# panbanda/islands

Measured on AMD Instinct MI355X. Metric: queries/sec @ recall@10>=0.95, 10Mx768 ef=128, higher is better.
Workload: dtype f32; 1 GPU; 10000000 x 768 f32 rows resident in HBM (in-memory provider), hierarchical Gaussian mixture, graph by the harness (tools/synth.py::build_graph: k-means medoid levels flattened into one layer, diversified links, parent->child and reverse edges), deg<= 60 (mean 38.6), query batch 1024, k=10, ef=128, cosine; nodes=10000000, dim=768, query_batch=1024, k=10, ef=128, graph=harness, distinct_leaves=False, parallelism=single, searches_in_flight=32, distinct_batches=497, replayed_queries=1688

## Files before the change

### include/islands_amd.h

```cpp
#ifndef ISLANDS_AMD_H
#define ISLANDS_AMD_H

#include <stddef.h>
#include <stdint.h>

#ifdef __cplusplus
extern "C" {
#endif

#define ISL_ABI_VERSION 3

typedef int32_t isl_status;

enum {
  ISL_OK = 0,
  ISL_ERR_DIMENSION_MISMATCH = 1,
  ISL_ERR_EMPTY_COLLECTION = 2,
  ISL_ERR_INVALID_CONFIG = 3,
  ISL_ERR_INDEX_NOT_BUILT = 4,
  ISL_ERR_NODE_NOT_FOUND = 5,
  ISL_ERR_SERIALIZATION = 6,
  ISL_ERR_DESERIALIZATION = 7,
  ISL_ERR_IO = 8,
  ISL_ERR_HNSW = 9,
// ... 126 lines not shown
  uint64_t expansions;
  uint64_t edges;
  uint64_t evals;
  uint64_t pushes;
  uint64_t exact_path;
  uint64_t replayed;
  double kernel_ms;
  uint64_t encoded_nodes;
  uint64_t recompute_rounds;
  uint64_t allocations;
} isl_search_stats;

isl_status isl_index_prepare(isl_index* idx, uint64_t max_nq, uint64_t max_ef, uint64_t max_k,
                             int32_t lanes);

isl_status isl_search_batch(const isl_index* idx, const float* queries, uint64_t nq, uint64_t d,
                            uint64_t k, uint64_t ef, uint64_t* out_ids, float* out_dist,
                            uint32_t* out_count);
isl_status isl_search_batch_async(const isl_index* idx, const float* queries, uint64_t nq, uint64_t d,
                                  uint64_t k, uint64_t ef, uint64_t* out_ids, float* out_dist,
                                  uint32_t* out_count, uint64_t* token);
isl_status isl_search_batch_device(const isl_index* idx, const float* d_queries, uint64_t nq,
                                   uint64_t d, uint64_t k, uint64_t ef, uint64_t* d_out_ids,
                                   float* d_out_dist, uint32_t* d_out_count, void* stream);
isl_status isl_search_batch_device_async(const isl_index* idx, const float* d_queries, uint64_t nq,
                                         uint64_t d, uint64_t k, uint64_t ef, uint64_t* d_out_ids,
                                         float* d_out_dist, uint32_t* d_out_count, void* stream,
                                         uint64_t* token);
isl_status isl_search_wait_stats(const isl_index* idx, uint64_t token, isl_search_stats* stats);
isl_status isl_search_wait(const isl_index* idx, uint64_t token);
isl_status isl_search_stream_wait(const isl_index* idx, uint64_t token, void* stream);
isl_status isl_index_group_counters(const isl_index* idx, uint64_t* launches, uint64_t* shared_launches,
                                    uint64_t* shared_calls);
isl_status isl_search(const isl_index* idx, const float* query, uint64_t d, uint64_t k,
                      uint64_t* out_ids, float* out_dist, uint32_t* out_count);

isl_status isl_search_last_stats(const isl_index* idx, isl_search_stats* out);

#define ISL_MAX_ENTRY_SEEDS 65536ull
isl_status isl_index_select_entry_seeds(isl_index* idx, uint64_t count, uint64_t* out_ids, uint64_t* out_count);
isl_status isl_index_set_entry_seeds(isl_index* idx, const uint64_t* ids, uint64_t count);
isl_status isl_index_entry_seeds(const isl_index* idx, uint64_t* out, uint64_t cap, uint64_t* count);
isl_status isl_index_pick_entries(const isl_index* idx, const float* queries, uint64_t nq, uint64_t d,
                                  uint64_t* out_ids, int32_t mem, void* stream);

isl_status isl_distance(int32_t metric, const float* a, uint64_t na, const float* b, uint64_t nb,
                        float* out);
isl_status isl_distance_squared(int32_t metric, const float* a, uint64_t na, const float* b,
                                uint64_t nb, float* out);
isl_status isl_distance_batch(int32_t metric, const float* query, uint64_t d, const float* rows,
                              uint64_t n, uint64_t row_len, float* out, int32_t mem, int32_t device,
                              void* stream);
isl_status isl_normalize_rows(float* rows, uint64_t n, uint64_t d, int32_t mem, int32_t device,
                              void* stream);

isl_status isl_distance_matrix(int32_t metric, const float* queries, uint64_t nq, const float* rows,
                               uint64_t n, uint64_t d, float* out, int32_t mem, int32_t device,
                               void* stream);
isl_status isl_bruteforce_topk(int32_t metric, const float* queries, uint64_t nq, const float* rows,
                               uint64_t n, uint64_t d, uint64_t k, uint64_t* out_ids, float* out_dist,
                               uint32_t* out_count, int32_t mem, int32_t device, void* stream);

isl_status isl_merge_topk(uint64_t nlists, uint64_t nq, uint64_t k, const uint64_t* ids,
                          const float* scores, const uint32_t* counts, const uint64_t* id_base,
                          uint64_t top_k, uint64_t* out_ids, float* out_scores,
                          uint32_t* out_src, uint32_t* out_count, int32_t mem, int32_t device,
// ... 159 lines not shown
```

### islands_amd/_ffi.py

```python
from __future__ import annotations

import ctypes as C
import os

os.environ.setdefault("GPU_MAX_HW_QUEUES", "32")

_HERE = os.path.dirname(os.path.abspath(__file__))
LIB_PATH = os.environ.get("ISL_AMD_LIB") or os.path.join(_HERE, "lib", "libislands_amd.so")

u64, u32, i32, f32 = C.c_uint64, C.c_uint32, C.c_int32, C.c_float
P = C.POINTER


class LeannConfigC(C.Structure):
    _fields_ = [
        ("m", u64), ("m0", u64), ("ef_construction", u64), ("ml", C.c_double),
        ("max_layers", u64), ("metric", u32), ("ef_search", u64), ("beam_width", u64),
        ("prune_ratio", f32), ("pruning_strategy", u32), ("high_degree_pruning", C.c_uint8),
        ("hub_percentile", f32), ("is_compact", C.c_uint8), ("is_recompute", C.c_uint8),
    ]


class BertConfigC(C.Structure):
    _fields_ = [("vocab_size", u32), ("hidden", u32), ("layers", u32), ("heads", u32),
# ... 46 lines not shown
    "isl_index_len": (u64, [C.c_void_p]),
    "isl_index_is_empty": (i32, [C.c_void_p]),
    "isl_index_dimension": (i32, [C.c_void_p, P(u64)]),
    "isl_index_storage_bytes": (u64, [C.c_void_p]),
    "isl_index_is_recompute": (i32, [C.c_void_p]),
    "isl_index_is_compact": (i32, [C.c_void_p]),
    "isl_index_config": (i32, [C.c_void_p, P(LeannConfigC)]),
    "isl_index_entry_point": (i32, [C.c_void_p, P(u64)]),
    "isl_index_max_level": (u64, [C.c_void_p]),
    "isl_index_get_neighbors": (i32, [C.c_void_p, u64, P(P(u64)), P(C.c_size_t)]),
    "isl_index_upload": (i32, [C.c_void_p, i32]),
    "isl_set_embeddings": (i32, [C.c_void_p, C.c_void_p, u64, u64, i32, i32]),
    "isl_search_batch": (i32, [C.c_void_p, C.c_void_p, u64, u64, u64, u64, C.c_void_p,
                               C.c_void_p, C.c_void_p]),
    "isl_hnsw_from_bytes": (i32, [C.c_void_p, C.c_size_t, i32, P(C.c_void_p)]),
    "isl_distance_matrix_bf16": (i32, [i32, C.c_void_p, u64, C.c_void_p, u64, u64, C.c_void_p, i32, i32,
                                       C.c_void_p]),
    "isl_index_set_pq_codes": (i32, [C.c_void_p, C.c_void_p, C.c_void_p, u64, i32]),
    "isl_search_two_level_batch": (i32, [C.c_void_p, C.c_void_p, u64, u64, u64, u64, C.c_float,
                                         C.c_void_p, C.c_void_p, C.c_void_p]),
    "isl_search_two_level_batch_device": (i32, [C.c_void_p, C.c_void_p, u64, u64, u64, u64,
                                                C.c_float, C.c_void_p, C.c_void_p, C.c_void_p,
                                                C.c_void_p]),
    "isl_search_two_level_batch_device_async": (i32, [C.c_void_p, C.c_void_p, u64, u64, u64, u64,
                                                      C.c_float, C.c_void_p, C.c_void_p, C.c_void_p,
                                                      C.c_void_p, P(u64)]),
    "isl_search_batch_device": (i32, [C.c_void_p, C.c_void_p, u64, u64, u64, u64, C.c_void_p,
                                      C.c_void_p, C.c_void_p, C.c_void_p]),
    "isl_search_batch_device_async": (i32, [C.c_void_p, C.c_void_p, u64, u64, u64, u64, C.c_void_p,
                                            C.c_void_p, C.c_void_p, C.c_void_p, P(u64)]),
    "isl_search_wait": (i32, [C.c_void_p, u64]),
    "isl_search_stream_wait": (i32, [C.c_void_p, u64, C.c_void_p]),
    "isl_index_group_counters": (i32, [C.c_void_p, P(u64), P(u64), P(u64)]),
    "isl_shard_record_bytes": (u64, [u64, u64]),
    "isl_merge_topk_packed_async": (i32, [u64, u64, u64, C.c_void_p, u64, C.c_void_p, u64, C.c_void_p, C.c_void_p,
                                          C.c_void_p, C.c_void_p, C.c_void_p, i32, C.c_void_p]),
    "isl_shard_unique_id": (i32, [C.c_void_p]),
    "isl_shard_group_create": (i32, [i32, i32, i32, C.c_void_p, P(C.c_void_p)]),
    "isl_shard_group_create_host": (i32, [i32, i32, i32, C.c_void_p, C.c_void_p, P(C.c_void_p)]),
    "isl_shard_group_info": (i32, [C.c_void_p, P(i32), P(i32), P(i32), P(i32)]),
    "isl_shard_group_free": (None, [C.c_void_p]),
    "isl_sharded_searcher_new": (i32, [C.c_void_p, C.c_void_p, u64, C.c_void_p, i32, P(C.c_void_p)]),
    "isl_sharded_searcher_free": (None, [C.c_void_p]),
    "isl_sharded_prepare": (i32, [C.c_void_p, u64, u64, u64]),
    "isl_sharded_submit": (i32, [C.c_void_p, C.c_void_p, u64, u64, u64, u64, C.c_void_p, P(u64)]),
    "isl_sharded_result": (i32, [C.c_void_p, u64, P(C.c_void_p), P(C.c_void_p), P(C.c_void_p), P(C.c_void_p),
                                 P(SearchStatsC)]),
    "isl_sharded_search_batch": (i32, [C.c_void_p, C.c_void_p, u64, u64, u64, u64, C.c_void_p, C.c_void_p,
                                       C.c_void_p, C.c_void_p]),
    "isl_sharded_flags": (i32, [C.c_void_p, P(u32)]),
    "isl_search_wait_stats": (i32, [C.c_void_p, u64, P(SearchStatsC)]),
    "isl_search_batch_async": (i32, [C.c_void_p, C.c_void_p, u64, u64, u64, u64, C.c_void_p,
                                     C.c_void_p, C.c_void_p, P(u64)]),
    "isl_index_prepare": (i32, [C.c_void_p, u64, u64, u64, i32]),
    "isl_search": (i32, [C.c_void_p, C.c_void_p, u64, u64, C.c_void_p, C.c_void_p, C.c_void_p]),
    "isl_search_last_stats": (i32, [C.c_void_p, P(SearchStatsC)]),
    "isl_distance": (i32, [i32, C.c_void_p, u64, C.c_void_p, u64, P(f32)]),
    "isl_distance_squared": (i32, [i32, C.c_void_p, u64, C.c_void_p, u64, P(f32)]),
    "isl_distance_batch": (i32, [i32, C.c_void_p, u64, C.c_void_p, u64, u64, C.c_void_p, i32, i32,
                                 C.c_void_p]),
    "isl_normalize_rows": (i32, [C.c_void_p, u64, u64, i32, i32, C.c_void_p]),
    "isl_distance_matrix": (i32, [i32, C.c_void_p, u64, C.c_void_p, u64, u64, C.c_void_p, i32, i32,
                                  C.c_void_p]),
    "isl_bruteforce_topk": (i32, [i32, C.c_void_p, u64, C.c_void_p, u64, u64, u64, C.c_void_p,
                                  C.c_void_p, C.c_void_p, i32, i32, C.c_void_p]),
    "isl_row_sumsq_bf16": (i32, [C.c_void_p, u64, u64, C.c_void_p, i32, i32, C.c_void_p]),
# ... 99 lines not shown
```

### islands_amd/csrc/common.hpp

```cpp
#pragma once

#include <hip/hip_runtime.h>

#include <algorithm>
#include <cstdarg>
#include <cstdint>
#include <cstdlib>
#include <cstdio>
#include <cstring>
#include <atomic>
#include <chrono>
#include <mutex>
#include <string>
#include <thread>
#include <type_traits>
#include <vector>

#include "../../include/islands_amd.h"
#include "device_buffer.hpp"
#include "row_table.hpp"

namespace isl {

struct ErrorRecord {
// ... 24 lines not shown
  switch (metric) {
    case ISL_METRIC_COSINE: f(std::integral_constant<int, ISL_METRIC_COSINE>{}); break;
    case ISL_METRIC_EUCLIDEAN: f(std::integral_constant<int, ISL_METRIC_EUCLIDEAN>{}); break;
    case ISL_METRIC_DOT: f(std::integral_constant<int, ISL_METRIC_DOT>{}); break;
    default: f(std::integral_constant<int, ISL_METRIC_MANHATTAN>{}); break;
  }
}

isl_status use_device(int32_t device);
int device_cu_count(int32_t device);

struct SearchWorkspace {
  uint32_t slots = 0;
  uint32_t ovf_bits = 0;
  DeviceBuffer<uint32_t> ovf_tab;
  DeviceBuffer<uint32_t> status;
  DeviceBuffer<uint64_t> payload;
  DeviceBuffer<uint32_t> ctr;
  DeviceBuffer<uint32_t> ticket;
  DeviceBuffer<uint32_t> redo;
  DeviceBuffer<uint32_t> replay;
  DeviceBuffer<uint32_t> qsel;
  DeviceBuffer<uint32_t> qsel_h;
  DeviceBuffer<uint64_t> plog;
  DeviceBuffer<float> q_stage;
  DeviceBuffer<uint64_t> ids_stage;
  DeviceBuffer<float> dist_stage;
  DeviceBuffer<uint32_t> count_stage;
  PinnedBuffer<float> h_q;
  PinnedBuffer<uint64_t> h_ids;
  PinnedBuffer<float> h_dist;
  PinnedBuffer<uint32_t> h_count;
  hipStream_t stream = nullptr;
  hipEvent_t ev0 = nullptr, ev1 = nullptr, ev_in = nullptr, ev_done = nullptr;
  bool busy = false;
  bool waiting = false;
  bool enqueued = false;
  bool ticket_clean = false;
  bool publish_results = false;
  uint64_t token = 0;
  uint64_t nq_inflight = 0, k_inflight = 0;
  uint32_t ef_inflight = 0;
  bool fast_inflight = false;
  hipStream_t st_inflight = nullptr;
  uint64_t* u_ids = nullptr;
  float* u_dist = nullptr;
  uint32_t* u_count = nullptr;
  PinnedBuffer<uint32_t> h_status;
  PinnedBuffer<uint32_t> h_ctr;
  PinnedBuffer<uint32_t> h_head;
  DeviceBuffer<uint64_t> d_prof;
  DeviceBuffer<uint64_t> d_tline;
  DeviceBuffer<uint32_t> q_entry;
  DeviceBuffer<float> co_q;
  DeviceBuffer<uint64_t> co_ids;
  DeviceBuffer<float> co_dist;
  DeviceBuffer<uint32_t> co_cnt;
  DeviceBuffer<uint32_t> miss;
  DeviceBuffer<uint32_t> uniq;
  DeviceBuffer<uint32_t> uniq_count;
  uint64_t miss_cap = 0;
  uint64_t pref_cap = 0;
  DeviceBuffer<uint32_t> qstate;
  DeviceBuffer<uint32_t> qflag;
  DeviceBuffer<uint32_t> qlist;
  PinnedBuffer<uint32_t> h_qlist;
  DeviceBuffer<uint32_t> uslots;
  DeviceBuffer<uint32_t> xslot;
  PinnedBuffer<uint32_t> h_xlist;
  DeviceBuffer<float> tl_tables;
  std::thread* worker = nullptr;
  bool threaded = false;
  isl_status worker_status = ISL_OK;
  ErrorRecord worker_error;
  uint64_t alloc_events = 0;
  uint64_t alloc_mark = 0;
  isl_search_stats stats{};
  bool grp = false;
  SearchWorkspace* grp_launch = nullptr;
  uint32_t grp_offset = 0;
  hipEvent_t grp_ready = nullptr;
  uint64_t grp_allocs = 0;
  bool grp_failed = false;
  isl_status grp_status = ISL_OK;
  ErrorRecord grp_error;
  int32_t pool_lane = -1;
  bool union_launch = false;
  PinnedBuffer<uint64_t> h_members;
  DeviceBuffer<uint32_t> grp_scratch;
};

constexpr int kSearchLanes = 32;

int hw_queues_at_load();
constexpr int kGroupBelowQueues = 8;
struct GroupSwitches { bool off; uint32_t cap, room; };
inline GroupSwitches group_switches() {
  auto num = [](const char* name) -> uint32_t {
    const char* e = getenv(name);
    const long long v = e ? atoll(e) : 0;
    return v > 0 ? (uint32_t)std::min<long long>(v, 0x7FFFFFFF) : 0u;
  };
  const char* off = getenv("ISL_NO_GROUP");
  const bool is_off = (off && *off) ? strcmp(off, "0") != 0 : hw_queues_at_load() >= kGroupBelowQueues;
  return GroupSwitches{is_off, num("ISL_GROUP_CAP"), num("ISL_GROUP_ROOM")};
}
struct GroupState;

struct ExactPool {
  uint32_t slots = 0;
  uint64_t cand_cap = 0;
  DeviceBuffer<float> cand_d;
  DeviceBuffer<uint32_t> cand_id;
  DeviceBuffer<uint32_t> vis_bits;
  uint64_t vis_words = 0;
  DeviceBuffer<uint32_t> ulist;
  uint32_t ulist_cap = 0;
  DeviceBuffer<uint32_t> locks;
  DeviceBuffer<uint32_t> xstate;
  uint32_t xstate_words = 0;
// ... 122 lines not shown
```

### islands_amd/csrc/search.hip

```cpp
#include "search_geometry.hpp"
#include "search_internal.hpp"

using namespace isl_lane;

namespace {

__global__ void fill_u32_kernel(uint32_t* p, uint64_t n, uint32_t v) {
  uint64_t i = (uint64_t)blockIdx.x * blockDim.x + threadIdx.x;
  uint64_t stride = (uint64_t)gridDim.x * blockDim.x;
  for (; i < n; i += stride) p[i] = v;
}

struct PublishParams {
  const uint32_t* src[6];
  uint32_t* dst[6];
  uint32_t words[6];
  uint32_t ticket_seg;
};
__global__ void publish_kernel(PublishParams pp) {
  const uint32_t seg = blockIdx.y;
  const uint32_t n = pp.words[seg];
  const uint32_t* __restrict__ src = pp.src[seg];
  uint32_t* __restrict__ dst = pp.dst[seg];
  for (uint32_t i = blockIdx.x * blockDim.x + threadIdx.x; i < n; i += gridDim.x * blockDim.x) {
    dst[i] = src[i];
    if (seg == pp.ticket_seg) const_cast<uint32_t*>(src)[i] = 0u;
  }
}
__global__ void copy_u128_kernel(const uint4* __restrict__ src, uint4* __restrict__ dst, uint64_t n) {
  for (uint64_t i = (uint64_t)blockIdx.x * blockDim.x + threadIdx.x; i < n; i += (uint64_t)gridDim.x * blockDim.x)
    dst[i] = src[i];
}
__global__ void copy_u32_kernel(const uint32_t* __restrict__ src, uint32_t* __restrict__ dst, uint64_t n) {
  for (uint64_t i = (uint64_t)blockIdx.x * blockDim.x + threadIdx.x; i < n; i += (uint64_t)gridDim.x * blockDim.x)
    dst[i] = src[i];
}

__global__ void seed_redo_kernel(const uint32_t* __restrict__ list, uint32_t n, uint32_t* __restrict__ redo,
                                 uint32_t* __restrict__ ticket) {
  for (uint32_t i = threadIdx.x; i < n; i += blockDim.x) redo[i] = list[i];
  if (threadIdx.x == 0) ticket[1] = n;
}

constexpr uint32_t kExactSlots = 32;
constexpr uint32_t kOvfBits = 15;


hipStream_t pool_stream(int32_t device, uint32_t lane, bool* created) {
  static std::mutex mu;
  static hipStream_t pool[64][32];
  static const uint32_t size = [] {
    const char* e = getenv("ISL_MAX_STREAMS");
    const int v = e ? atoi(e) : 16;
    return (uint32_t)std::min(std::max(v, 1), 32);
  }();
  *created = false;
  if (device < 0 || device >= 64) return nullptr;
  std::lock_guard<std::mutex> lock(mu);
  hipStream_t& st = pool[device][lane % size];
  if (!st) {
    if (hipStreamCreateWithFlags(&st, hipStreamNonBlocking) != hipSuccess) { (void)hipGetLastError(); st = nullptr; }
    else *created = true;
  }
  return st;
}

}

isl_status isl_lane::ensure_lane_stream(const isl_index* idx, isl::SearchWorkspace& ws) {
  if (ws.stream) return ISL_OK;
  bool created = false;
  hipStream_t st = pool_stream(idx->device, ws.pool_lane >= 0 ? (uint32_t)ws.pool_lane : (uint32_t)(&ws - idx->ws), &created);
  if (!st) return isl::fail(ISL_ERR_DEVICE, "hipStreamCreate failed for a search lane");
  if (created) ws.alloc_events++;
  if (!ws.ev_done) { ISL_HIP(hipEventCreateWithFlags(&ws.ev_done, hipEventDisableTiming)); ws.alloc_events++; }
  if (!ws.ev0) { ISL_HIP(hipEventCreate(&ws.ev0)); ws.alloc_events++; }
  if (!ws.ev1) { ISL_HIP(hipEventCreate(&ws.ev1)); ws.alloc_events++; }
  if (!ws.ev_in) { ISL_HIP(hipEventCreateWithFlags(&ws.ev_in, hipEventDisableTiming)); ws.alloc_events++; }
  if (!ws.ticket) {
    ISL_TRY(ws.ticket.reserve(16, &ws.alloc_events));
    ws.ticket_clean = false;
  }
  ISL_TRY(ws.h_head.reserve(16, &ws.alloc_events));
  ws.stream = st;
  return ISL_OK;
}

void isl_lane::copy_words(const uint32_t* src, uint32_t* dst, uint64_t n, uint32_t grid, uint32_t block, hipStream_t st) {
  hipLaunchKernelGGL(copy_u32_kernel, dim3(grid), dim3(block), 0, st, src, dst, n);
}

isl_status isl_lane::prepare_workspace(const isl_index* idx, isl::SearchWorkspace& ws, uint32_t nq, uint32_t slots,
                                       uint32_t plog_cap) {
  ISL_TRY(ensure_lane_stream(idx, ws));
  uint64_t* const ev = &ws.alloc_events;
  const uint64_t cap = nq < 1024 ? 1024 : nq;
  ISL_TRY(ws.h_status.reserve(cap, ev));
  ISL_TRY(ws.h_ctr.reserve(cap * 4, ev));
  if (ws.slots < slots || !ws.ovf_tab) {
    ws.ovf_tab.reset();
    ws.slots = 0;
    static const uint32_t ovf_bits_cfg = [] {
      const char* e = getenv("ISL_OVF_BITS");
      const int v = e ? atoi(e) : (int)kOvfBits;
      return (uint32_t)std::min(15, std::max(10, v));
    }();
    ws.ovf_bits = ovf_bits_cfg;
    uint64_t n = (uint64_t)slots << ovf_bits_cfg;
    ISL_TRY(ws.ovf_tab.reserve(n, ev));
    hipLaunchKernelGGL(fill_u32_kernel, dim3(2048), dim3(256), 0, ws.stream, ws.ovf_tab, n, EMPTY);
    ISL_HIP(hipGetLastError());
    ISL_HIP(hipStreamSynchronize(ws.stream));
    ws.slots = slots;
  }
  ISL_TRY(ws.status.reserve(cap, ev));
  ISL_TRY(ws.payload.reserve(cap, ev));
  ISL_TRY(ws.ctr.reserve(cap * 4, ev));
// ... 341 lines not shown
  tl_last_stats.st = st;
}

}

isl_status isl_lane::search_enqueue(const isl_index* idx, isl::SearchWorkspace& ws, const SearchCall& c,
                                      const RoundPlan& plan, bool warm) {
  const isl_status st = search_enqueue_impl(idx, ws, c, plan, warm);
  if (st != ISL_OK) {
    const isl::ErrorRecord keep = isl::last_error();
    hipStream_t s = call_stream(ws, c);
    if (c.mode == StreamMode::USER || s) (void)hipStreamSynchronize(s);
    (void)hipGetLastError();
    ws.ticket_clean = false;
    ws.enqueued = false;
    isl::last_error() = keep;
  }
  return st;
}

isl_status isl_lane::search_finish(const isl_index* idx, isl::SearchWorkspace& ws, uint32_t* misses,
                                     bool defer_statuses) {
  if (!ws.enqueued) return isl::fail(ISL_ERR_INVALID_ARGUMENT, "no search in flight for this token");
  ws.enqueued = false;
  const uint64_t nq = ws.nq_inflight;
  const bool use_fast = ws.fast_inflight;
  const isl::SearchWorkspace& lw = ws.grp_launch ? *ws.grp_launch : ws;
  ISL_HIP(hipEventSynchronize(lw.ev_done));
  const uint32_t* status = ws.h_status;
  const uint32_t* ctr = ws.h_ctr;
  const uint32_t* head = ws.h_head;
  isl::DeviceBuffer<uint64_t> d_prof = std::move(ws.d_prof);
  float ms = 0.0f;
  (void)hipEventElapsedTime(&ms, lw.ev0, lw.ev1);

  isl_search_stats& ss = ws.stats;
  ss = isl_search_stats{};
  ss.queries = nq;
  ss.exact_path = head[1];
  ss.replayed = head[3];
  ss.kernel_ms = ms;
  ss.allocations = ws.alloc_events - ws.alloc_mark + ws.grp_allocs;
  for (uint64_t i = 0; i < nq; i++) {
    ss.expansions += ctr[i * 4 + 0];
    ss.edges += ctr[i * 4 + 1];
    ss.evals += ctr[i * 4 + 2];
    ss.pushes += ctr[i * 4 + 3];
  }
  if (use_fast && !idx->recompute && !misses && nq >= 16)
    idx->evals_hint.store(((uint64_t)ws.ef_inflight << 32) | std::min<uint64_t>(ss.evals / nq, 0xFFFFFFFFull),
                          std::memory_order_relaxed);
  if (ws.d_tline) {
    std::vector<uint64_t> tl(nq * 2 + 2);
    tl[0] = 0x154C494E45ull;
    tl[1] = nq;
    ISL_HIP(hipMemcpy(tl.data() + 2, ws.d_tline, nq * 16, hipMemcpyDeviceToHost));
    ws.d_tline.reset();
    static std::mutex tl_mu;
    std::lock_guard<std::mutex> lock(tl_mu);
    if (FILE* f = fopen(getenv("ISL_TIMELINE"), "ab")) {
      fwrite(tl.data(), 8, tl.size(), f);
      fclose(f);
    }
  }
  if (d_prof) {
    std::vector<uint64_t> pr(nq * 8);
    ISL_HIP(hipMemcpy(pr.data(), d_prof, nq * 64, hipMemcpyDeviceToHost));
// ... 664 lines not shown
```

### islands_amd/csrc/search_group.hip

```cpp
#include <memory>

#include "search_geometry.hpp"
#include "search_group_plan.hpp"
#include "search_internal.hpp"

using namespace isl_lane;

namespace isl {

struct GroupState {
  isl_group::Planner plan;
  std::vector<std::unique_ptr<SearchWorkspace>> slots;
  SearchCall calls[kSearchLanes];
  uint64_t launches = 0, shared_launches = 0, shared_calls = 0;
};

}

namespace {

struct GroupMember {
  const float* q;
  uint64_t* ids;
  float* dist;
  uint32_t* count;
  uint32_t* h_status;
  uint32_t* h_ctr;
  uint32_t* h_head;
  uint32_t offset, nq;
};
static_assert(sizeof(GroupMember) == 64, "member table rows are eight words");

constexpr uint32_t kMaxMembers = isl::kSearchLanes;
constexpr uint32_t kScatterBlocks = 64;

__global__ void group_gather_kernel(const GroupMember* __restrict__ tab, float* __restrict__ dst, uint32_t d) {
  const GroupMember m = tab[blockIdx.y];
  const uint64_t n = (uint64_t)m.nq * d;
  const float* __restrict__ src = m.q;
  float* __restrict__ out = dst + (uint64_t)m.offset * d;
  const uint64_t t = (uint64_t)blockIdx.x * blockDim.x + threadIdx.x;
  const uint64_t stride = (uint64_t)gridDim.x * blockDim.x;
  if (n % 4 == 0 && (((uintptr_t)src | (uintptr_t)out) & 15) == 0) {
    const uint4* __restrict__ s4 = reinterpret_cast<const uint4*>(src);
    uint4* __restrict__ o4 = reinterpret_cast<uint4*>(out);
    for (uint64_t i = t; i < n / 4; i += stride) o4[i] = s4[i];
  } else {
// ... 67 lines not shown
  uint32_t* mine = sp.scratch + blockIdx.y * 4;
  if (lane == 0) {
    if (n_exact) atomicAdd(&mine[0], n_exact);
    if (n_replayed) atomicAdd(&mine[1], n_replayed);
  }
  __threadfence();
  __syncthreads();
  if (threadIdx.x != 0) return;
  if (atomicAdd(&mine[2], 1u) == gridDim.x - 1) {
    __threadfence();
    const uint32_t ex = atomicExch(&mine[0], 0u), rp = atomicExch(&mine[1], 0u);
    mine[2] = 0u;
    for (uint32_t i = 0; i < 16; ++i) m.h_head[i] = i == 1 ? ex : i == 3 ? rp : 0u;
  }
  uint32_t* all = sp.scratch + kMaxMembers * 4;
  if (atomicAdd(all, 1u) == gridDim.x * gridDim.y - 1) {
    *all = 0u;
    for (uint32_t i = 0; i < 16; ++i) {
      sp.h_head[i] = sp.ticket[i];
      sp.ticket[i] = 0u;
    }
  }
}

__global__ void zero_u32_kernel(uint32_t* p, uint32_t n) {
  for (uint32_t i = blockIdx.x * blockDim.x + threadIdx.x; i < n; i += gridDim.x * blockDim.x) p[i] = 0u;
}

uint32_t group_cap(const isl_index* idx) { return idx->group_sw.cap ? idx->group_sw.cap : isl_group::kDefaultCap; }

isl::GroupState& state_of(const isl_index* idx) {
  if (!idx->group) {
    idx->group = new isl::GroupState();
    idx->group->plan.configure(group_cap(idx), 0);
  }
  return *idx->group;
}

isl_status prepare_slot(const isl_index* idx, isl::SearchWorkspace& gw, uint64_t nq, uint64_t d, uint64_t k) {
  uint64_t* const ev = &gw.alloc_events;
  gw.union_launch = true;
  ISL_TRY(ensure_lane_stream(idx, gw));
  ISL_TRY(gw.q_stage.reserve(nq * d, ev));
  const uint64_t outs = nq * std::max<uint64_t>(k, 1);
  ISL_TRY(gw.ids_stage.reserve(outs, ev));
  ISL_TRY(gw.dist_stage.reserve(outs, ev));
  ISL_TRY(gw.count_stage.reserve(nq, ev));
  ISL_TRY(gw.h_members.reserve((uint64_t)kMaxMembers * 8, ev));
  if (!gw.grp_scratch) {
    ISL_TRY(gw.grp_scratch.reserve(kMaxMembers * 4 + 4, ev));
    hipLaunchKernelGGL(zero_u32_kernel, dim3(1), dim3(256), 0, gw.stream, gw.grp_scratch.get(), kMaxMembers * 4 + 4);
    ISL_HIP(hipGetLastError());
  }
  return ISL_OK;
}

isl::SearchWorkspace& slot(isl::GroupState& g, int32_t w) {
  if (!g.slots[w]) {
    g.slots[w].reset(new isl::SearchWorkspace());
    g.slots[w]->pool_lane = isl::kSearchLanes - 1 - w;
  }
  return *g.slots[w];
}

void grow_slots(const isl_index* idx, isl::GroupState& g, uint32_t n) {
  if (g.slots.size() < n) g.slots.resize(n);
  g.plan.configure(group_cap(idx), n);
}

isl_status enqueue_alone(const isl_index* idx, isl::GroupState& g, const isl_group::Launch& L) {
  const uint32_t lane_no = L.members[0].call;
  isl::SearchWorkspace& ws = idx->ws[lane_no];
  SearchCall c = g.calls[lane_no];
  c.user_stream = nullptr;
  c.mode = StreamMode::OWN_AFTER_EVENT;
  ISL_TRY(search_enqueue(idx, ws, c));
  ws.grp_launch = nullptr;
  ws.grp_offset = 0;
  ws.grp_ready = ws.ev1;
  return ISL_OK;
}

isl_status enqueue_group_impl(const isl_index* idx, isl::GroupState& g, const isl_group::Launch& L,
                              isl::SearchWorkspace& gw) {
  const uint64_t d = L.key.d, k = L.key.k;
  const uint32_t nm = (uint32_t)L.members.size();
  if (nm > kMaxMembers) return isl::fail(ISL_ERR_SEARCH, "Search error: %u calls in one group launch", nm);
  CallGeometry cg;
  ISL_TRY(call_geometry(idx, d, k, L.key.ef, nullptr, cg));
  ISL_TRY(prepare_slot(idx, gw, L.nq, d, k));
  ISL_TRY(prepare_workspace(idx, gw, L.nq, (uint32_t)std::min<uint64_t>(L.nq, cg.lane_slots), cg.plog_cap));
  GroupMember* tab = reinterpret_cast<GroupMember*>(gw.h_members.get());
  for (uint32_t i = 0; i < nm; ++i) {
    const isl_group::Member& mb = L.members[i];
    isl::SearchWorkspace& ws = idx->ws[mb.call];
    const SearchCall& c = g.calls[mb.call];
    ISL_TRY(ws.h_status.reserve(std::max<uint64_t>(mb.nq, 1024), &ws.alloc_events));
    ISL_TRY(ws.h_ctr.reserve(std::max<uint64_t>(mb.nq, 1024) * 4, &ws.alloc_events));
    tab[i] = GroupMember{c.queries, c.ids, c.dist, c.count, ws.h_status, ws.h_ctr, ws.h_head, mb.offset, mb.nq};
    ISL_HIP(hipStreamWaitEvent(gw.stream, ws.ev_in, 0));
  }
  hipLaunchKernelGGL(group_gather_kernel, dim3(64, nm), dim3(256), 0, gw.stream, tab, gw.q_stage.get(), (uint32_t)d);
  ISL_HIP(hipGetLastError());
  SearchCall u;
  u.queries = gw.q_stage;
  u.nq = L.nq;
  u.d = d;
  u.k = k;
  u.ef = L.key.ef;
  u.ids = gw.ids_stage;
  u.dist = gw.dist_stage;
  u.count = gw.count_stage;
  u.mode = StreamMode::OWN;
  ISL_TRY(search_enqueue(idx, gw, u));
  ScatterParams sp{};
  sp.tab = tab;
  sp.ids = gw.ids_stage;
  sp.dist = gw.dist_stage;
  sp.count = gw.count_stage;
  sp.status = gw.status;
  sp.ctr = gw.ctr;
  sp.redo = gw.redo;
  sp.plog = reinterpret_cast<const uint2*>(gw.plog.get());
  sp.ticket = gw.ticket;
  sp.h_head = gw.h_head;
  sp.scratch = gw.grp_scratch;
  sp.k = (uint32_t)k;
  sp.ef = cg.ef;
  sp.plog_cap = cg.plog_cap;
  hipLaunchKernelGGL(group_scatter_kernel, dim3(kScatterBlocks, nm), dim3(256), 0, gw.stream, sp);
  ISL_HIP(hipGetLastError());
  gw.ticket_clean = true;
  ISL_HIP(hipEventRecord(gw.ev_done, gw.stream));
  return ISL_OK;
}

isl_status enqueue_group(const isl_index* idx, isl::GroupState& g, const isl_group::Launch& L) {
  isl::SearchWorkspace& gw = slot(g, L.workspace);
  const uint64_t mark = gw.alloc_events;
  const isl_status st = enqueue_group_impl(idx, g, L, gw);
  gw.enqueued = false;
  if (st != ISL_OK) {
    const isl::ErrorRecord keep = isl::last_error();
    if (gw.stream) (void)hipStreamSynchronize(gw.stream);
    (void)hipGetLastError();
    gw.ticket_clean = false;
    isl::last_error() = keep;
    return st;
  }
  for (const isl_group::Member& mb : L.members) {
    isl::SearchWorkspace& ws = idx->ws[mb.call];
    ws.grp_launch = &gw;
    ws.grp_offset = mb.offset;
    ws.grp_ready = gw.ev_done;
    ws.grp_allocs = gw.alloc_events - mark;
    ws.enqueued = true;
    ws.nq_inflight = mb.nq;
    ws.k_inflight = L.key.k;
    ws.ef_inflight = gw.ef_inflight;
    ws.fast_inflight = gw.fast_inflight;
    ws.st_inflight = gw.stream;
  }
  return ISL_OK;
}

void poll(const isl_index* idx, isl::GroupState& g) {
  for (const isl_group::Planner::Live& l : g.plan.live()) {
    hipEvent_t ev = l.workspace >= 0 ? g.slots[l.workspace]->ev_done : idx->ws[l.first_call].ev_done;
    const hipError_t e = hipEventQuery(ev);
    if (e == hipSuccess) g.plan.complete(l.id);
    else (void)hipGetLastError();
  }
}

void submit(const isl_index* idx, isl::GroupState& g, uint32_t wanted) {
  isl_group::Launch L;
  for (;;) {
    if (wanted != isl_group::kNone && !g.plan.held(wanted)) wanted = isl_group::kNone;
    if (!g.plan.next(wanted, L)) break;
    const isl_status st = L.workspace < 0 ? enqueue_alone(idx, g, L) : enqueue_group(idx, g, L);
    if (st == ISL_OK) {
      g.launches += 1;
      if (L.workspace >= 0) { g.shared_launches += 1; g.shared_calls += L.members.size(); }
      continue;
    }
    for (const isl_group::Member& mb : L.members) {
      isl::SearchWorkspace& ws = idx->ws[mb.call];
      ws.grp_failed = true;
      ws.grp_status = st;
      ws.grp_error = isl::last_error();
      ws.grp_launch = nullptr;
      ws.enqueued = false;
    }
    g.plan.abandon(L.id);
  }
}

}

bool isl_lane::group_takes(const isl_index* idx, const SearchCall& c) {
  static const bool instrumented = getenv("ISL_TIMELINE") != nullptr || getenv("ISL_DEBUG") != nullptr;
  isl_group::CallTraits t;
  t.device_async = true;
  t.recompute = idx->recompute;
  t.two_level = c.two_level;
  t.hnsw = idx->is_hnsw;
  t.construction = idx->build_q_entry != nullptr;
  t.instrumented = instrumented;
  t.nq = c.nq;
  return isl_group::groupable(t, idx->group_sw.off, group_cap(idx));
}

isl_status isl_lane::group_arrive(const isl_index* idx, isl::SearchWorkspace& ws, const SearchCall& c) {
  CallGeometry cg;
  ISL_TRY(call_geometry(idx, c.d, c.k, c.ef, nullptr, cg));
  ISL_TRY(ensure_lane_stream(idx, ws));
  ISL_HIP(hipEventRecord(ws.ev_in, c.user_stream));
  const uint32_t lane_no = (uint32_t)(&ws - idx->ws);
  std::lock_guard<std::mutex> lock(idx->group_mu);
  isl::GroupState& g = state_of(idx);
  if (g.slots.empty()) grow_slots(idx, g, isl::kSearchLanes / 2);
  g.calls[lane_no] = c;
  ws.grp = true;
  ws.grp_failed = false;
  ws.grp_launch = nullptr;
  ws.grp_allocs = 0;
  poll(idx, g);
  const uint32_t room = idx->group_sw.room ? idx->group_sw.room : cg.slots;
  g.plan.arrive(lane_no, (uint32_t)c.nq, isl_group::Key{c.d, c.k, cg.ef}, room);
  submit(idx, g, isl_group::kNone);
  if (ws.grp_failed) {
    ws.grp = false;
    isl::last_error() = ws.grp_error;
    return ws.grp_status;
  }
  return ISL_OK;
}

void isl_lane::group_pump(const isl_index* idx) {
  std::lock_guard<std::mutex> lock(idx->group_mu);
  if (!idx->group || !idx->group->plan.any_held()) return;
  poll(idx, *idx->group);
  submit(idx, *idx->group, isl_group::kNone);
}

isl_status isl_lane::group_before_wait(const isl_index* idx, isl::SearchWorkspace& ws) {
  std::lock_guard<std::mutex> lock(idx->group_mu);
  isl::GroupState& g = state_of(idx);
  poll(idx, g);
  submit(idx, g, (uint32_t)(&ws - idx->ws));
  if (ws.grp_failed) {
    isl::last_error() = ws.grp_error;
    return ws.grp_status;
  }
  return ISL_OK;
}

void isl_lane::group_after_wait(const isl_index* idx, isl::SearchWorkspace& ws) {
  std::lock_guard<std::mutex> lock(idx->group_mu);
  if (!idx->group) return;
  isl::GroupState& g = *idx->group;
  const isl::ErrorRecord keep = isl::last_error();
  g.plan.finished((uint32_t)(&ws - idx->ws));
  ws.grp = false;
  ws.grp_launch = nullptr;
  if (g.plan.any_held()) {
    poll(idx, g);
    submit(idx, g, isl_group::kNone);
  }
  isl::last_error() = keep;
}

isl_status isl_lane::group_prepare(const isl_index* idx, uint64_t max_nq, uint64_t max_ef, uint64_t max_k, int32_t lanes,
                                   uint32_t ovf_waves, uint32_t plog_cap) {
  if (idx->group_sw.off || idx->recompute || idx->is_hnsw || idx->build_q_entry) return ISL_OK;
  std::lock_guard<std::mutex> lock(idx->group_mu);
  isl::GroupState& g = state_of(idx);
  const uint32_t cap = group_cap(idx);
  const uint32_t n = isl_group::workspaces_for((uint32_t)lanes, max_nq, cap);
  const uint64_t nq = isl_group::workspace_queries((uint32_t)lanes, max_nq, cap);
  grow_slots(idx, g, std::max<uint32_t>(n, (uint32_t)g.slots.size()));
  const uint64_t d = idx->rows.d();
  for (uint32_t w = 0; w < n; ++w) {
    isl::SearchWorkspace& gw = slot(g, (int32_t)w);
    ISL_TRY(prepare_slot(idx, gw, nq, d, std::max<uint64_t>(max_k, 1)));
    ISL_TRY(prepare_workspace(idx, gw, (uint32_t)nq, (uint32_t)std::min<uint64_t>(nq, ovf_waves), plog_cap));
    if (idx->seeds.count()) ISL_TRY(gw.q_entry.reserve(nq * 4, &gw.alloc_events));
  }
  for (int round = 0; round < 2; ++round) {
    for (uint32_t w = 0; w < n; ++w) {
      isl::SearchWorkspace& gw = *g.slots[w];
      GroupMember* tab = reinterpret_cast<GroupMember*>(gw.h_members.get());
      tab[0] = GroupMember{};
      hipLaunchKernelGGL(group_gather_kernel, dim3(1, 1), dim3(256), 0, gw.stream, tab, gw.q_stage.get(), (uint32_t)d);
      ISL_HIP(hipGetLastError());
      SearchCall warm_call;
      warm_call.d = d;
      warm_call.k = std::min<uint64_t>(max_k, max_ef);
// ... 6 lines not shown
      sp.count = gw.count_stage;
      sp.status = gw.status;
      sp.ctr = gw.ctr;
      sp.redo = gw.redo;
      sp.plog = reinterpret_cast<const uint2*>(gw.plog.get());
      sp.ticket = gw.ticket;
      sp.h_head = gw.h_head;
      sp.scratch = gw.grp_scratch;
      sp.k = (uint32_t)std::max<uint64_t>(max_k, 1);
      sp.ef = (uint32_t)max_ef;
      sp.plog_cap = plog_cap;
      tab[0].h_head = gw.h_head;
      hipLaunchKernelGGL(group_scatter_kernel, dim3(kScatterBlocks, 1), dim3(256), 0, gw.stream, sp);
      ISL_HIP(hipGetLastError());
      gw.ticket_clean = true;
      ISL_HIP(hipEventRecord(gw.ev_done, gw.stream));
    }
    for (uint32_t w = 0; w < n; ++w) ISL_HIP(hipStreamSynchronize(g.slots[w]->stream));
  }
  return ISL_OK;
}

extern "C" isl_status isl_index_group_counters(const isl_index* idx, uint64_t* launches, uint64_t* shared_launches,
                                               uint64_t* shared_calls) {
  if (!idx) return isl::fail(ISL_ERR_INVALID_ARGUMENT, "index is NULL");
  std::lock_guard<std::mutex> lock(idx->group_mu);
  const isl::GroupState* g = idx->group;
  if (launches) *launches = g ? g->launches : 0;
  if (shared_launches) *shared_launches = g ? g->shared_launches : 0;
  if (shared_calls) *shared_calls = g ? g->shared_calls : 0;
  return ISL_OK;
}

void isl::free_group_state(isl_index* idx) {
  std::lock_guard<std::mutex> lock(idx->group_mu);
  GroupState* g = idx->group;
  if (!g) return;
  for (int i = 0; i < kSearchLanes; ++i)
    if (g->plan.held((uint32_t)i)) submit(idx, *g, (uint32_t)i);
  for (auto& s : g->slots)
    if (s) {
      if (s->stream) (void)hipStreamSynchronize(s->stream);
      (void)hipGetLastError();
      free_workspace(*s);
    }
  delete g;
  idx->group = nullptr;
}
```

### islands_amd/csrc/search_group_plan.hpp

```cpp
#pragma once

#include <algorithm>
#include <cstdint>
#include <vector>

namespace isl_group {

constexpr uint32_t kNone = 0xFFFFFFFFu;
constexpr uint32_t kDefaultCap = 4096;

struct Key {
  uint64_t d = 0, k = 0, ef = 0;
  bool operator==(const Key& o) const { return d == o.d && k == o.k && ef == o.ef; }
};

struct CallTraits {
  bool device_async = false;
  bool recompute = false;
  bool two_level = false;
  bool hnsw = false;
  bool construction = false;
  bool instrumented = false;
  uint64_t nq = 0;
};
inline bool groupable(const CallTraits& t, bool grouping_off, uint32_t cap) {
  return !grouping_off && t.device_async && !t.recompute && !t.two_level && !t.hnsw && !t.construction &&
         !t.instrumented && t.nq >= 1 && t.nq <= cap;
}

inline uint32_t workspaces_for(uint32_t lanes, uint64_t max_nq, uint32_t cap) {
  if (lanes < 2 || cap == 0) return 0;
  const uint64_t by_queries = ((uint64_t)lanes * max_nq + cap - 1) / cap + 1;
  return (uint32_t)std::min<uint64_t>(by_queries, lanes / 2);
}
inline uint64_t workspace_queries(uint32_t lanes, uint64_t max_nq, uint32_t cap) {
  return std::min<uint64_t>(cap, (uint64_t)lanes * max_nq);
}

struct Member {
  uint32_t call = 0;
  uint32_t nq = 0;
  uint32_t offset = 0;
};
struct Launch {
  uint32_t id = 0;
  int32_t workspace = -1;
  Key key{};
  uint32_t nq = 0;
  std::vector<Member> members;
};

class Planner {
 public:
  void configure(uint32_t cap, uint32_t workspaces) {
    cap_ = std::max<uint32_t>(cap, 1);
    if (workspaces > ws_busy_.size()) ws_busy_.resize(workspaces, false);
  }
  uint32_t cap() const { return cap_; }
  uint32_t workspaces() const { return (uint32_t)ws_busy_.size(); }
  uint64_t inflight() const { return inflight_; }
  bool held(uint32_t call) const {
    for (const Held& h : held_) if (h.call == call) return true;
    return false;
  }
  bool any_held() const { return !held_.empty(); }

  void arrive(uint32_t call, uint32_t nq, const Key& key, uint32_t room) { held_.push_back(Held{call, nq, key, room}); }

  bool next(uint32_t wanted, Launch& out) {
    if (wanted != kNone) {
      for (const Held& h : held_)
        if (h.call == wanted) return take(h.key, true, wanted, out);
      return false;
    }
    std::vector<Key> seen;
    for (size_t i = 0; i < held_.size(); ++i) {
      const Key key = held_[i].key;
      if (std::find(seen.begin(), seen.end(), key) != seen.end()) continue;
      seen.push_back(key);
      uint64_t total = 0;
      for (const Held& h : held_) if (h.key == key) total += h.nq;
      if ((total >= cap_ || inflight_ < held_[i].room) && take(key, false, kNone, out)) return true;
    }
    return false;
  }

  struct Live { uint32_t id; int32_t workspace; uint32_t first_call; };
  std::vector<Live> live() const {
    std::vector<Live> v;
    for (const Flight& f : flights_) if (!f.complete) v.push_back(Live{f.id, f.workspace, f.calls.front()});
    return v;
  }
  void complete(uint32_t launch) {
    for (size_t i = 0; i < flights_.size(); ++i)
      if (flights_[i].id == launch) { settle(i); return; }
  }
  int32_t finished(uint32_t call) {
    for (size_t i = 0; i < flights_.size(); ++i) {
      Flight& f = flights_[i];
      auto it = std::find(f.calls.begin(), f.calls.end(), call);
      if (it == f.calls.end()) continue;
      f.calls.erase(it);
      if (!f.complete) { f.complete = true; inflight_ -= f.nq; }
      if (!f.calls.empty()) return -1;
      const int32_t w = f.workspace;
      if (w >= 0) ws_busy_[w] = false;
      flights_.erase(flights_.begin() + i);
      return w;
    }
    return -1;
  }
  void abandon(uint32_t launch) {
    for (size_t i = 0; i < flights_.size(); ++i)
      if (flights_[i].id == launch) {
        Flight& f = flights_[i];
        if (!f.complete) inflight_ -= f.nq;
        if (f.workspace >= 0) ws_busy_[f.workspace] = false;
        flights_.erase(flights_.begin() + i);
        return;
      }
  }
  void drop(uint32_t call) {
    for (size_t i = 0; i < held_.size(); ++i)
      if (held_[i].call == call) { held_.erase(held_.begin() + i); return; }
  }

 private:
  struct Held { uint32_t call, nq; Key key; uint32_t room; };
  struct Flight { uint32_t id; int32_t workspace; uint32_t nq; bool complete; std::vector<uint32_t> calls; };

  void settle(size_t i) {
    Flight& f = flights_[i];
    if (f.complete) return;
    f.complete = true;
    inflight_ -= f.nq;
  }
  int32_t free_workspace() const {
    for (size_t w = 0; w < ws_busy_.size(); ++w) if (!ws_busy_[w]) return (int32_t)w;
    return -1;
  }
  bool take(const Key& key, bool forced, uint32_t wanted, Launch& out) {
    std::vector<size_t> pick;
    uint64_t total = 0;
    for (size_t i = 0; i < held_.size(); ++i) {
      if (!(held_[i].key == key)) continue;
      if (!pick.empty() && total + held_[i].nq > cap_) break;
      pick.push_back(i);
      total += held_[i].nq;
    }
    if (pick.empty()) return false;
    int32_t w = -1;
    if (pick.size() > 1) {
      w = free_workspace();
      if (w < 0) {
        if (!forced) return false;
        pick.clear();
        for (size_t i = 0; i < held_.size(); ++i) if (held_[i].call == wanted) pick.push_back(i);
      }
    }
    out = Launch{};
    out.id = next_id_++;
    out.workspace = pick.size() > 1 ? w : -1;
    out.key = key;
    Flight f{out.id, out.workspace, 0, false, {}};
    for (size_t i : pick) {
      out.members.push_back(Member{held_[i].call, held_[i].nq, out.nq});
      out.nq += held_[i].nq;
      f.calls.push_back(held_[i].call);
    }
    f.nq = out.nq;
    for (size_t n = pick.size(); n-- > 0;) held_.erase(held_.begin() + pick[n]);
    if (out.workspace >= 0) ws_busy_[out.workspace] = true;
    inflight_ += out.nq;
    flights_.push_back(f);
    return true;
  }

  uint32_t cap_ = kDefaultCap;
  uint32_t next_id_ = 1;
  uint64_t inflight_ = 0;
  std::vector<Held> held_;
  std::vector<Flight> flights_;
  std::vector<bool> ws_busy_;
};

}
```

### islands_amd/csrc/search_internal.hpp

```cpp
#pragma once

#include "common.hpp"

namespace isl_lane __attribute__((visibility("hidden"))) {

enum class StreamMode { OWN, USER, OWN_AFTER_USER, OWN_AFTER_EVENT };

struct SearchCall {
  const float* queries = nullptr;
  uint64_t nq = 0, d = 0, k = 0, ef = 0;
  uint64_t* ids = nullptr;
  float* dist = nullptr;
  uint32_t* count = nullptr;
  hipStream_t user_stream = nullptr;
  StreamMode mode = StreamMode::OWN;
  bool two_level = false;
  float ratio = 0.0f;
};
inline hipStream_t call_stream(const isl::SearchWorkspace& ws, const SearchCall& c) {
  return c.mode == StreamMode::USER ? c.user_stream : ws.stream;
}

struct RoundPlan {
  uint32_t active = 0;
  uint32_t exact = 0;
  bool exact_parks = false;
  bool listed = false;
  uint32_t prefetch = 0;
  uint32_t retry = 0;
  uint32_t window_scale = 1;
  bool tables_built = false;
};

isl_status ensure_lane_stream(const isl_index* idx, isl::SearchWorkspace& ws);
isl_status ensure_pool(const isl_index* idx, isl::SearchWorkspace& ws);
void copy_words(const uint32_t* src, uint32_t* dst, uint64_t n, uint32_t grid, uint32_t block, hipStream_t st);
isl_status prepare_workspace(const isl_index* idx, isl::SearchWorkspace& ws, uint32_t nq, uint32_t slots,
                             uint32_t plog_cap);
isl_status search_enqueue(const isl_index* idx, isl::SearchWorkspace& ws, const SearchCall& c,
                          const RoundPlan& plan = RoundPlan{}, bool warm = false);
isl_status search_finish(const isl_index* idx, isl::SearchWorkspace& ws, uint32_t* misses = nullptr,
                         bool defer_statuses = false);
isl_status search_statuses(isl::SearchWorkspace& ws, uint64_t nq);
isl_status search_sync(const isl_index* idx, isl::SearchWorkspace& ws, const SearchCall& c);

isl_status prepare_recompute(isl::SearchWorkspace& ws, uint64_t nq, uint64_t state_words_per_query);
isl_status tl_retry_short(isl::SearchWorkspace& ws, uint64_t nq, uint32_t& window_scale, uint32_t* nshort);
isl_status recompute_rounds(const isl_index* idx, isl::SearchWorkspace& ws, const SearchCall& c);
isl_status recompute_coalesced(const isl_index* idx, isl::SearchWorkspace& ws, const SearchCall& c);

bool group_takes(const isl_index* idx, const SearchCall& c);
isl_status group_arrive(const isl_index* idx, isl::SearchWorkspace& ws, const SearchCall& c);
void group_pump(const isl_index* idx);
isl_status group_before_wait(const isl_index* idx, isl::SearchWorkspace& ws);
void group_after_wait(const isl_index* idx, isl::SearchWorkspace& ws);
isl_status group_prepare(const isl_index* idx, uint64_t max_nq, uint64_t max_ef, uint64_t max_k, int32_t lanes,
                         uint32_t ovf_waves, uint32_t plog_cap);

}
```

Baseline: 1.647 million queries/s.

## Place grouped search launches on least-loaded pooled streams

Grouped search launches are now assigned to a stream from the pool chosen by the planner as the one with the fewest in-flight queries, instead of always using the lane's own stream. The aim is to spread concurrent searches across hardware queues so launches do not serialize on one busy stream. The pool is capped below the hardware queue count, and per-stream placement counters plus a query API are added. Kernel timing for shared launches is read once per launch. Risks include extra stream rebinding and event ordering subtleties when lanes switch streams.

Result: no change. 1.649 million queries/s (median of 2 runs) (+0.1%).

```diff
diff --git a/include/islands_amd.h b/include/islands_amd.h
--- a/include/islands_amd.h
+++ b/include/islands_amd.h
@@ -182,6 +182,8 @@
 isl_status isl_search_stream_wait(const isl_index* idx, uint64_t token, void* stream);
 isl_status isl_index_group_counters(const isl_index* idx, uint64_t* launches, uint64_t* shared_launches,
                                     uint64_t* shared_calls);
+isl_status isl_index_group_placement(const isl_index* idx, uint32_t n_max, uint32_t* n, uint64_t* launches_per_stream,
+                                     uint64_t* queries_per_stream);
 isl_status isl_search(const isl_index* idx, const float* query, uint64_t d, uint64_t k,
                       uint64_t* out_ids, float* out_dist, uint32_t* out_count);
 
diff --git a/islands_amd/_ffi.py b/islands_amd/_ffi.py
--- a/islands_amd/_ffi.py
+++ b/islands_amd/_ffi.py
@@ -102,6 +102,7 @@
     "isl_search_wait": (i32, [C.c_void_p, u64]),
     "isl_search_stream_wait": (i32, [C.c_void_p, u64, C.c_void_p]),
     "isl_index_group_counters": (i32, [C.c_void_p, P(u64), P(u64), P(u64)]),
+    "isl_index_group_placement": (i32, [C.c_void_p, u32, P(u32), P(u64), P(u64)]),
     "isl_shard_record_bytes": (u64, [u64, u64]),
     "isl_merge_topk_packed_async": (i32, [u64, u64, u64, C.c_void_p, u64, C.c_void_p, u64, C.c_void_p, C.c_void_p,
                                           C.c_void_p, C.c_void_p, C.c_void_p, i32, C.c_void_p]),
diff --git a/islands_amd/csrc/common.hpp b/islands_amd/csrc/common.hpp
--- a/islands_amd/csrc/common.hpp
+++ b/islands_amd/csrc/common.hpp
@@ -80,6 +80,7 @@
   PinnedBuffer<float> h_dist;
   PinnedBuffer<uint32_t> h_count;
   hipStream_t stream = nullptr;
+  bool lane_set_up = false;
   hipEvent_t ev0 = nullptr, ev1 = nullptr, ev_in = nullptr, ev_done = nullptr;
   bool busy = false;
   bool waiting = false;
@@ -134,6 +135,8 @@
   ErrorRecord grp_error;
   int32_t pool_lane = -1;
   bool union_launch = false;
+  bool launch_ms_read = false;
+  float launch_ms = 0.0f;
   PinnedBuffer<uint64_t> h_members;
   DeviceBuffer<uint32_t> grp_scratch;
 };
diff --git a/islands_amd/csrc/search.hip b/islands_amd/csrc/search.hip
--- a/islands_amd/csrc/search.hip
+++ b/islands_amd/csrc/search.hip
@@ -46,14 +46,21 @@
 constexpr uint32_t kOvfBits = 15;
 
 
+uint32_t pool_size() {
+  static const uint32_t size = [] {
+    const char* e = getenv("ISL_MAX_STREAMS");
+    const int v = e ? atoi(e) : 16;
+    uint32_t n = (uint32_t)std::min(std::max(v, 1), 32);
+    const int q = isl::hw_queues_at_load();
+    if (q < isl::kGroupBelowQueues) n = std::min<uint32_t>(n, (uint32_t)std::max(q - 1, 1));
+    return n;
+  }();
+  return size;
+}
 hipStream_t pool_stream(int32_t device, uint32_t lane, bool* created) {
   static std::mutex mu;
   static hipStream_t pool[64][32];
-  static const uint32_t size = [] {
-    const char* e = getenv("ISL_MAX_STREAMS");
-    const int v = e ? atoi(e) : 16;
-    return (uint32_t)std::min(std::max(v, 1), 32);
-  }();
+  const uint32_t size = pool_size();
   *created = false;
   if (device < 0 || device >= 64) return nullptr;
   std::lock_guard<std::mutex> lock(mu);
@@ -67,12 +74,21 @@
 
 }
 
-isl_status isl_lane::ensure_lane_stream(const isl_index* idx, isl::SearchWorkspace& ws) {
-  if (ws.stream) return ISL_OK;
+uint32_t isl_lane::placement_streams() { return std::min<uint32_t>(pool_size(), (uint32_t)std::max(isl::hw_queues_at_load(), 1)); }
+
+isl_status isl_lane::set_call_stream(const isl_index* idx, isl::SearchWorkspace& ws, int32_t placement) {
   bool created = false;
-  hipStream_t st = pool_stream(idx->device, ws.pool_lane >= 0 ? (uint32_t)ws.pool_lane : (uint32_t)(&ws - idx->ws), &created);
+  const uint32_t own = ws.pool_lane >= 0 ? (uint32_t)ws.pool_lane : (uint32_t)(&ws - idx->ws);
+  hipStream_t st = pool_stream(idx->device, placement >= 0 ? (uint32_t)placement : own, &created);
   if (!st) return isl::fail(ISL_ERR_DEVICE, "hipStreamCreate failed for a search lane");
   if (created) ws.alloc_events++;
+  ws.stream = st;
+  return ISL_OK;
+}
+
+isl_status isl_lane::ensure_lane_stream(const isl_index* idx, isl::SearchWorkspace& ws) {
+  if (ws.stream && ws.lane_set_up) return ISL_OK;
+  if (!ws.stream) ISL_TRY(set_call_stream(idx, ws, -1));
   if (!ws.ev_done) { ISL_HIP(hipEventCreateWithFlags(&ws.ev_done, hipEventDisableTiming)); ws.alloc_events++; }
   if (!ws.ev0) { ISL_HIP(hipEventCreate(&ws.ev0)); ws.alloc_events++; }
   if (!ws.ev1) { ISL_HIP(hipEventCreate(&ws.ev1)); ws.alloc_events++; }
@@ -82,7 +98,7 @@
     ws.ticket_clean = false;
   }
   ISL_TRY(ws.h_head.reserve(16, &ws.alloc_events));
-  ws.stream = st;
+  ws.lane_set_up = true;
   return ISL_OK;
 }
 
@@ -490,7 +506,17 @@
   const uint32_t* head = ws.h_head;
   isl::DeviceBuffer<uint64_t> d_prof = std::move(ws.d_prof);
   float ms = 0.0f;
-  (void)hipEventElapsedTime(&ms, lw.ev0, lw.ev1);
+  if (ws.grp_launch) {
+    std::lock_guard<std::mutex> lock(idx->group_mu);
+    isl::SearchWorkspace& gw = *ws.grp_launch;
+    if (!gw.launch_ms_read) {
+      (void)hipEventElapsedTime(&gw.launch_ms, gw.ev0, gw.ev1);
+      gw.launch_ms_read = true;
+    }
+    ms = gw.launch_ms;
+  } else {
+    (void)hipEventElapsedTime(&ms, lw.ev0, lw.ev1);
+  }
 
   isl_search_stats& ss = ws.stats;
   ss = isl_search_stats{};
diff --git a/islands_amd/csrc/search_group.hip b/islands_amd/csrc/search_group.hip
--- a/islands_amd/csrc/search_group.hip
+++ b/islands_amd/csrc/search_group.hip
@@ -13,6 +13,7 @@
   std::vector<std::unique_ptr<SearchWorkspace>> slots;
   SearchCall calls[kSearchLanes];
   uint64_t launches = 0, shared_launches = 0, shared_calls = 0;
+  uint64_t placed_launches[32] = {}, placed_queries[32] = {};
 };
 
 }
@@ -146,9 +147,13 @@
 isl::GroupState& state_of(const isl_index* idx) {
   if (!idx->group) {
     idx->group = new isl::GroupState();
-    idx->group->plan.configure(group_cap(idx), 0);
+    idx->group->plan.configure(group_cap(idx), 0, placement_streams());
   }
   return *idx->group;
+}
+
+isl_status place(const isl_index* idx, isl::GroupState& g, isl::SearchWorkspace& ws, const isl_group::Launch& L) {
+  return set_call_stream(idx, ws, g.plan.queues() ? (int32_t)L.queue : -1);
 }
 
 isl_status prepare_slot(const isl_index* idx, isl::SearchWorkspace& gw, uint64_t nq, uint64_t d, uint64_t k) {
@@ -179,7 +184,7 @@
 
 void grow_slots(const isl_index* idx, isl::GroupState& g, uint32_t n) {
   if (g.slots.size() < n) g.slots.resize(n);
-  g.plan.configure(group_cap(idx), n);
+  g.plan.configure(group_cap(idx), n, placement_streams());
 }
 
 isl_status enqueue_alone(const isl_index* idx, isl::GroupState& g, const isl_group::Launch& L) {
@@ -188,6 +193,7 @@
   SearchCall c = g.calls[lane_no];
   c.user_stream = nullptr;
   c.mode = StreamMode::OWN_AFTER_EVENT;
+  ISL_TRY(place(idx, g, ws, L));
   ISL_TRY(search_enqueue(idx, ws, c));
   ws.grp_launch = nullptr;
   ws.grp_offset = 0;
@@ -252,8 +258,10 @@
 isl_status enqueue_group(const isl_index* idx, isl::GroupState& g, const isl_group::Launch& L) {
   isl::SearchWorkspace& gw = slot(g, L.workspace);
   const uint64_t mark = gw.alloc_events;
-  const isl_status st = enqueue_group_impl(idx, g, L, gw);
+  isl_status st = place(idx, g, gw, L);
+  if (st == ISL_OK) st = enqueue_group_impl(idx, g, L, gw);
   gw.enqueued = false;
+  gw.launch_ms_read = false;
   if (st != ISL_OK) {
     const isl::ErrorRecord keep = isl::last_error();
     if (gw.stream) (void)hipStreamSynchronize(gw.stream);
@@ -296,6 +304,7 @@
     if (st == ISL_OK) {
       g.launches += 1;
       if (L.workspace >= 0) { g.shared_launches += 1; g.shared_calls += L.members.size(); }
+      if (L.queue < g.plan.queues() && L.queue < 32) { g.placed_launches[L.queue] += 1; g.placed_queries[L.queue] += L.nq; }
       continue;
     }
     for (const isl_group::Member& mb : L.members) {
@@ -345,6 +354,7 @@
   submit(idx, g, isl_group::kNone);
   if (ws.grp_failed) {
     ws.grp = false;
+    (void)set_call_stream(idx, ws, -1);
     isl::last_error() = ws.grp_error;
     return ws.grp_status;
   }
@@ -378,6 +388,7 @@
   g.plan.finished((uint32_t)(&ws - idx->ws));
   ws.grp = false;
   ws.grp_launch = nullptr;
+  if (ws.stream) (void)set_call_stream(idx, ws, -1);
   if (g.plan.any_held()) {
     poll(idx, g);
     submit(idx, g, isl_group::kNone);
@@ -450,6 +461,21 @@
   return ISL_OK;
 }
 
+extern "C" isl_status isl_index_group_placement(const isl_index* idx, uint32_t n_max, uint32_t* n, uint64_t* launches_per_stream,
+                                                uint64_t* queries_per_stream) {
+  if (!idx) return isl::fail(ISL_ERR_INVALID_ARGUMENT, "index is NULL");
+  if (n_max && (!launches_per_stream || !queries_per_stream)) return isl::fail(ISL_ERR_INVALID_ARGUMENT, "NULL buffer");
+  std::lock_guard<std::mutex> lock(idx->group_mu);
+  const isl::GroupState* g = idx->group;
+  const uint32_t streams = g ? std::min<uint32_t>(g->plan.queues(), 32) : 0;
+  if (n) *n = streams;
+  for (uint32_t i = 0; i < n_max; ++i) {
+    launches_per_stream[i] = i < streams ? g->placed_launches[i] : 0;
+    queries_per_stream[i] = i < streams ? g->placed_queries[i] : 0;
+  }
+  return ISL_OK;
+}
+
 void isl::free_group_state(isl_index* idx) {
   std::lock_guard<std::mutex> lock(idx->group_mu);
   GroupState* g = idx->group;
diff --git a/islands_amd/csrc/search_group_plan.hpp b/islands_amd/csrc/search_group_plan.hpp
--- a/islands_amd/csrc/search_group_plan.hpp
+++ b/islands_amd/csrc/search_group_plan.hpp
@@ -48,17 +48,21 @@
   Key key{};
   uint32_t nq = 0;
   std::vector<Member> members;
+  uint32_t queue = 0;
 };
 
 class Planner {
  public:
-  void configure(uint32_t cap, uint32_t workspaces) {
+  void configure(uint32_t cap, uint32_t workspaces, uint32_t queues = 0) {
     cap_ = std::max<uint32_t>(cap, 1);
     if (workspaces > ws_busy_.size()) ws_busy_.resize(workspaces, false);
+    if (queues > load_.size()) load_.resize(queues, 0);
   }
   uint32_t cap() const { return cap_; }
   uint32_t workspaces() const { return (uint32_t)ws_busy_.size(); }
   uint64_t inflight() const { return inflight_; }
+  uint32_t queues() const { return (uint32_t)load_.size(); }
+  uint64_t load(uint32_t queue) const { return queue < load_.size() ? load_[queue] : 0; }
   bool held(uint32_t call) const {
     for (const Held& h : held_) if (h.call == call) return true;
     return false;
@@ -101,7 +105,7 @@
       auto it = std::find(f.calls.begin(), f.calls.end(), call);
       if (it == f.calls.end()) continue;
       f.calls.erase(it);
-      if (!f.complete) { f.complete = true; inflight_ -= f.nq; }
+      settle(i);
       if (!f.calls.empty()) return -1;
       const int32_t w = f.workspace;
       if (w >= 0) ws_busy_[w] = false;
@@ -114,7 +118,7 @@
     for (size_t i = 0; i < flights_.size(); ++i)
       if (flights_[i].id == launch) {
         Flight& f = flights_[i];
-        if (!f.complete) inflight_ -= f.nq;
+        settle(i);
         if (f.workspace >= 0) ws_busy_[f.workspace] = false;
         flights_.erase(flights_.begin() + i);
         return;
@@ -127,13 +131,19 @@
 
  private:
   struct Held { uint32_t call, nq; Key key; uint32_t room; };
-  struct Flight { uint32_t id; int32_t workspace; uint32_t nq; bool complete; std::vector<uint32_t> calls; };
+  struct Flight { uint32_t id; int32_t workspace; uint32_t nq; bool complete; std::vector<uint32_t> calls; uint32_t queue; };
 
   void settle(size_t i) {
     Flight& f = flights_[i];
     if (f.complete) return;
     f.complete = true;
     inflight_ -= f.nq;
+    if (f.queue < load_.size()) load_[f.queue] -= f.nq;
+  }
+  uint32_t least_loaded() const {
+    uint32_t best = 0;
+    for (uint32_t q = 1; q < load_.size(); ++q) if (load_[q] < load_[best]) best = q;
+    return best;
   }
   int32_t free_workspace() const {
     for (size_t w = 0; w < ws_busy_.size(); ++w) if (!ws_busy_[w]) return (int32_t)w;
@@ -162,7 +172,8 @@
     out.id = next_id_++;
     out.workspace = pick.size() > 1 ? w : -1;
     out.key = key;
-    Flight f{out.id, out.workspace, 0, false, {}};
+    out.queue = least_loaded();
+    Flight f{out.id, out.workspace, 0, false, {}, out.queue};
     for (size_t i : pick) {
       out.members.push_back(Member{held_[i].call, held_[i].nq, out.nq});
       out.nq += held_[i].nq;
@@ -172,6 +183,7 @@
     for (size_t n = pick.size(); n-- > 0;) held_.erase(held_.begin() + pick[n]);
     if (out.workspace >= 0) ws_busy_[out.workspace] = true;
     inflight_ += out.nq;
+    if (out.queue < load_.size()) load_[out.queue] += out.nq;
     flights_.push_back(f);
     return true;
   }
@@ -182,6 +194,7 @@
   std::vector<Held> held_;
   std::vector<Flight> flights_;
   std::vector<bool> ws_busy_;
-};
-
-}
+  std::vector<uint64_t> load_;
+};
+
+}
diff --git a/islands_amd/csrc/search_internal.hpp b/islands_amd/csrc/search_internal.hpp
--- a/islands_amd/csrc/search_internal.hpp
+++ b/islands_amd/csrc/search_internal.hpp
@@ -33,6 +33,8 @@
 };
 
 isl_status ensure_lane_stream(const isl_index* idx, isl::SearchWorkspace& ws);
+uint32_t placement_streams();
+isl_status set_call_stream(const isl_index* idx, isl::SearchWorkspace& ws, int32_t placement);
 isl_status ensure_pool(const isl_index* idx, isl::SearchWorkspace& ws);
 void copy_words(const uint32_t* src, uint32_t* dst, uint64_t n, uint32_t grid, uint32_t block, hipStream_t st);
 isl_status prepare_workspace(const isl_index* idx, isl::SearchWorkspace& ws, uint32_t nq, uint32_t slots,
```
